# NetSys/demi

Measured on AMD Instinct MI355X. Metric: candidate schedules evaluated/sec on Raft-5 fuzz (RandomScheduler executions), higher is better.
Workload: dtype u8

## Files before the change

demi_amd/csrc/demi_device.hpp:

```cpp
#pragma once

#ifndef __HIPCC_RTC__
#include <hip/hip_runtime.h>
#include <stdint.h>
#endif

#include "../../include/demi_gpu.h"

namespace demi {

struct DevModel {
  uint32_t n_actors, n_msg_types, n_classes, code_len;
  uint32_t inv_kind, inv_fa, inv_va, inv_fb;
  uint32_t fp_match_mask, wide ;
  uint32_t n_timer_types;
  uint32_t timer_types;
  uint32_t meta[DEMI_MAX_MSG_TYPES];
  uint32_t handler_start[DEMI_MAX_CLASSES * DEMI_MAX_MSG_TYPES];
  uint32_t actor_class[DEMI_MAX_ACTORS];
  uint64_t init_state[DEMI_MAX_ACTORS];
  uint32_t divmagic[257];
  uint32_t arr_len;
  uint32_t optab[64];
  uint32_t code[DEMI_MAX_CODE];
// ... 125 lines not shown
__device__ __forceinline__ void pairs_clear(PairSet& p) { p.w = 0; }
__device__ __forceinline__ uint32_t pairs_get(const PairSet& p, uint32_t a, uint32_t b) { return (uint32_t)(p.w >> (a * 8 + b)) & 1u; }
__device__ __forceinline__ void pairs_put(PairSet& p, uint32_t a, uint32_t b, bool on) {
  if (on) p.w |= 1ULL << (a * 8 + b); else p.w &= ~(1ULL << (a * 8 + b));
}
#endif
struct Net {
  uint32_t inaccessible, killed;
  PairSet partitioned;
};
__device__ __forceinline__ bool crosses_partition(const Net& n, uint32_t snd, uint32_t rcv) {
  if (snd == rcv && !((n.killed >> snd) & 1)) return false;
#ifdef DEMI_BIG
  const uint32_t part = pairs_get(n.partitioned, snd, rcv) | pairs_get(n.partitioned, rcv, snd);
#else
  const uint32_t part = (uint32_t)((n.partitioned.w >> (snd * 8 + rcv)) | (n.partitioned.w >> (rcv * 8 + snd))) & 1u;
#endif
  return (part | (n.inaccessible >> rcv) | (n.inaccessible >> snd)) & 1u;
}

#ifdef DEMI_BIG
#ifndef DEMI_JIT_TYPE_OF_TIX
#define DEMI_JIT_TYPE_OF_TIX 0u
#endif
__device__ __forceinline__ uint32_t tq_pack(uint32_t rcv, uint32_t type, uint32_t tix) { (void)type; return (rcv << 2) | tix; }
__device__ __forceinline__ uint32_t tq_rcv(uint32_t b) { return b >> 2; }
__device__ __forceinline__ uint32_t tq_type(uint32_t b) { return ((uint32_t)(DEMI_JIT_TYPE_OF_TIX) >> (5u * (b & 3u))) & 31u; }
#else
__device__ __forceinline__ uint32_t tq_pack(uint32_t rcv, uint32_t type, uint32_t tix) { (void)tix; return (rcv << 5) | type; }
__device__ __forceinline__ uint32_t tq_rcv(uint32_t b) { return b >> 5; }
__device__ __forceinline__ uint32_t tq_type(uint32_t b) { return b & 31u; }
#endif

__device__ __forceinline__ void hash_step(uint64_t& h, uint64_t v) { h = (h ^ v) * 0x100000001B3ULL; }

__device__ __forceinline__ uint32_t fld(uint64_t s, uint32_t f) { return (uint32_t)(s >> (8 * f)) & 0xFF; }
__device__ __forceinline__ uint32_t state_field(const uint64_t* st, uint32_t a, uint32_t f) {
#ifdef DEMI_WIDE
  return (uint32_t)(st[(ST_WORDS * a + (f >> 2)) * 64] >> (16 * (f & 3))) & 0xFFFFu;
#else
  return (uint32_t)(st[(ST_WORDS * a) * 64] >> (8 * f)) & 0xFFu;
#endif
}
__device__ __forceinline__ uint32_t arr_load(const uint64_t* st, uint32_t a, uint32_t idx) {
  if (ARR_LEN == 0 || idx >= ARR_LEN) return 0;
  const unsigned char* w = reinterpret_cast<const unsigned char*>(st + (size_t)(ST_WORDS * a + FLD_WORDS + idx / (WIDE_TU ? 4u : 8u)) * 64);
  if (WIDE_TU) return reinterpret_cast<const uint16_t*>(w)[idx & 3u];
  return w[idx & 7u];
}
__device__ __forceinline__ void arr_store(uint64_t* st, uint32_t a, uint32_t idx, uint32_t v) {
  if (ARR_LEN == 0 || idx >= ARR_LEN) return;
  unsigned char* w = reinterpret_cast<unsigned char*>(st + (size_t)(ST_WORDS * a + FLD_WORDS + idx / (WIDE_TU ? 4u : 8u)) * 64);
  if (WIDE_TU) reinterpret_cast<uint16_t*>(w)[idx & 3u] = (uint16_t)v;
  else w[idx & 7u] = (unsigned char)v;
}


}
```

demi_amd/csrc/demi_gpu.hip:

```cpp
#include <hip/hip_runtime.h>

#include <cstdarg>
#include <cstdio>
#include <cstring>
#include <algorithm>
#include <memory>
#include <new>
#include <queue>
#include <string>
#include <type_traits>
#include <unordered_map>
#include <unordered_set>
#include <vector>
#include <chrono>

#include "../../include/demi_gpu.h"
#include "knobs.hpp"
#include "devbuf.hpp"
#include "k1_random_explore.hpp"
#include "k2_replay.hpp"
#include "k2_removal_round.hpp"
#include "k2_wildcard.hpp"
#include "k2_wildcard_cand.hpp"
#include "k2_wildcard_round.hpp"
// ... 548 lines not shown
  ctx->have_dpor = false;
  return DEMI_OK;
}

static bool is_big(const DevModel& h) { return h.n_actors > DEMI_MAX_ACTORS; }
static uint32_t jit_k1_hot();
static uint32_t jit_k1s_hot() {
  return demi_host::knob("DEMI_JIT_K1S_HOT") ? (uint32_t)demi_host::knob_int("DEMI_JIT_K1S_HOT", 0, 64, 0) : jit_k1_hot();
}
static uint32_t jit_k1_hot() {
  return (uint32_t)demi_host::knob_int("DEMI_JIT_K1_HOT", 0, 64, 0);
}

static uint32_t jit_k3_hot(const DevModel& h);
static std::string jit_source(const DevModel& h, int kernel) {
  std::string src =
      "typedef unsigned char uint8_t; typedef unsigned short uint16_t; typedef unsigned int uint32_t;\n"
      "typedef unsigned long uint64_t; typedef int int32_t; typedef long int64_t; typedef unsigned long size_t; typedef unsigned long uintptr_t;\n"
      "#include \"sim_core.hpp\"\n";
  char defs[512];
  snprintf(defs, sizeof defs, "#define DEMI_PEND_HOT %u\n#define DEMI_K1_HOT %u\n#define DEMI_JIT_A %uu\n#define DEMI_JIT_INV_KIND %uu\n#define DEMI_JIT_INV_FA %uu\n"
           "#define DEMI_JIT_INV_VA %uu\n#define DEMI_JIT_INV_FB %uu\n#define DEMI_JIT_FP_MASK 0x%xu\n"
           "#define DEMI_JIT_NTT %uu\n#define DEMI_JIT_TIMER_TYPES 0x%xu\n#define DEMI_JIT_TIX_PACKED 0x%llxull\n#define DEMI_JIT_NT %uu\n",
           (unsigned)(kernel == JK_K3 ? jit_k3_hot(h)  : h.wide ? DEMI_PEND_HOT / 2 : DEMI_PEND_HOT), (unsigned)((kJit[kernel].flags & JF_SPREAD) ? jit_k1s_hot() : jit_k1_hot()), h.n_actors, h.inv_kind, h.inv_fa, h.inv_va, h.inv_fb, h.fp_match_mask,
           h.n_timer_types, h.timer_types, (unsigned long long)h.tix_packed, h.n_msg_types);
  src = defs + src;
  if (h.inv_kind & DEMI_INV_PROGRAM) src = "#define DEMI_JIT_INV_PROG 1\n" + src;
  if (h.wide) src = "#define DEMI_WIDE 1\n" + src;
  if (is_big(h)) {
    uint32_t type_of_tix = 0;
    for (uint32_t t = 0; t < h.n_msg_types; t++) if ((h.timer_types >> t) & 1u) type_of_tix |= t << (5u * (h.meta[t] >> 8));
    src = "#define DEMI_BIG 1\n#define DEMI_JIT_TYPE_OF_TIX " + std::to_string(type_of_tix) + "u\n" + src;
  }
  if (h.npay > 2) src = "#define DEMI_JIT_NPAY " + std::to_string(h.npay) + "\n" + src;
  if (h.arr_len) src = "#define DEMI_JIT_ARR_LEN " + std::to_string(h.arr_len) + "u\n" + src;
  {
    bool crash = false, rnd = false;
    for (uint32_t pc = 0; pc < h.code_len; pc++) { crash |= (h.code[pc] & 0xFFu) == DEMI_OP_CRASH; rnd |= (h.code[pc] & 0x3Fu) == DEMI_OP_RND; }
    if (!crash) src = "#define DEMI_JIT_NO_CRASH 1\n" + src;
    if (!rnd) src = "#define DEMI_JIT_NO_RND 1\n" + src;
  }
  if (const char* d = demi_host::knob("DEMI_JIT_DEFINES")) {
    std::string extra, item;
    for (const char* c = d;; c++) {
      if (*c == ';' || *c == '\0') {
        if (!item.empty()) { const size_t eq = item.find('='); extra += "#define " + (eq == std::string::npos ? item : item.substr(0, eq) + " " + item.substr(eq + 1)) + "\n"; }
        item.clear();
        if (*c == '\0') break;
      } else item += *c;
    }
    src = extra + src;
  }
  if (const long x = demi_host::knob_int("DEMI_JIT_K1_WAVES_PER_EU", 1, 8, 0))
    src = "#define DEMI_K1_MIN_WAVES_PER_EU " + std::to_string(x) + "\n" + src;
  src += demi_jit::generate_vm(h, jk_is_k1(kernel) && !jk_k1_records(kernel) && !demi_host::knob("DEMI_JIT_NO_FX_SCHED"));
  src += "#define DEMI_VM_RUN vm_run_jit\n#include \"";
  src += kJit[kernel].include;
  src += "\"\n";
  if (kJit[kernel].args) src += std::string("template __global__ void ") + kJit[kernel].name + "(const " + kJit[kernel].args + ");\n";
  return src;
}

static int jit_compile(demi_ctx* ctx, const DevModel& h, int kernel, std::vector<char>& image, std::string& name) {
#ifdef DEMI_NO_JIT_SOURCES
  return fail(ctx, DEMI_ERR_DEVICE, "specialisation failed: this library was built without the embedded kernel sources "
                                    "(build it with __graft_entry__.build())");
// ... 3923 lines not shown
```

demi_amd/csrc/jit.hpp:

```cpp
#pragma once
#include "knobs.hpp"

#include <dlfcn.h>

#include <algorithm>
#include <cstdio>
#include <cstdlib>
#include <cstring>
#include <string>
#include <vector>

#include "sim_core.hpp"

namespace demi_jit {

struct FxSchedule {
  bool ok = false;
  std::vector<uint32_t> cls;
  std::vector<int32_t> slot;
};
enum : uint32_t { FXK_SEND = 0, FXK_CANCEL = 1, FXK_TSET = 2, FXK_CRASH = 3 };
inline uint32_t fx_class_of(uint32_t row) {
  const uint32_t op = row & 0x3Fu, type = (row >> 17) & 0x7Fu;
  if (op == DEMI_OP_SEND || op == DEMI_OP_BCAST) return FXK_SEND << 16;
// ... 135 lines not shown
    if (is_fx(pc)) {
      const uint32_t c = fx_class_of(h.code[pc]);
      int32_t j = next;
      while (j < (int32_t)S.cls.size() && S.cls[j] != c) j++;
      if (j >= (int32_t)S.cls.size()) { S.cls.push_back(c); j = (int32_t)S.cls.size() - 1; }
      S.slot[pc] = j;
      next = j + 1;
    }
    uint32_t o[2];
    const int k = succ(pc, o);
    for (int i = 0; i < k; i++) if (o[i] < n) lo[o[i]] = std::max(lo[o[i]], next);
  }
  {
    std::vector<int32_t> used(S.cls.size(), 0), remap(S.cls.size(), -1);
    for (uint32_t pc = 0; pc < n; pc++) if (S.slot[pc] >= 0) used[S.slot[pc]] = 1;
    std::vector<uint32_t> cls2;
    for (size_t j = 0; j < S.cls.size(); j++) if (used[j]) { remap[j] = (int32_t)cls2.size(); cls2.push_back(S.cls[j]); }
    for (uint32_t pc = 0; pc < n; pc++) if (S.slot[pc] >= 0) S.slot[pc] = remap[S.slot[pc]];
    S.cls.swap(cls2);
  }
  S.ok = S.cls.size() <= DEMI_FX_CAP;
  return S;
}

inline uint32_t k1_fxq_slots(const demi::DevModel& h, bool sched) {
  if (!sched) return DEMI_FX_CAP;
  const FxSchedule fxs = fx_schedule(h);
  if (!fxs.ok) return DEMI_FX_CAP;
  uint32_t nq = 0;
  for (uint32_t c : fxs.cls) nq += (c >> 16) == FXK_SEND;
  return nq ? nq : 1u;
}

inline std::string generate_vm(const demi::DevModel& h, bool sched = false) {
  using namespace demi;
  std::string s;
  char buf[512];
  auto emit = [&](const char* fmt, auto... a) { snprintf(buf, sizeof buf, fmt, a...); s += buf; };
  FxSchedule fxs;
  std::vector<uint32_t> fxq_of_slot;
  if (sched) fxs = fx_schedule(h);
  if (fxs.ok) {
    s += "#define DEMI_JIT_FX_SCHED 1\n#define DEMI_JIT_FX_APPLY";
    uint32_t nq = 0;
    for (size_t j = 0; j < fxs.cls.size(); j++) {
      const uint32_t c = fxs.cls[j], type = c & 0xFFu;
      const bool snd = (c >> 16) == FXK_SEND;
      emit(" DEMI_FX_SLOT(%zu, %uu, %uu, %uu, %uu, %uu)", j, c >> 16, (c >> 8) & 0xFFu, type, snd ? 0u : (h.meta[type & 31u] >> 8), snd ? nq : 0u);
      fxq_of_slot.push_back(snd ? nq : 0u);
      if (snd) nq++;
    }
    emit("\n#define DEMI_JIT_FXQ_SLOTS %uu\n", nq ? nq : 1u);
  }
  s += "namespace demi {\n";
  const bool long_msg = h.npay > 2;
  const char* fx_pack_fn = long_msg ? "fx_pack_area" : "fx_pack";
  if (fxs.ok)
    s += std::string("#define DEMI_FX_AT(SLOT, Q, OP, TYPE, TGT, ...) { mem.fxq[(Q) * 64] = ") + fx_pack_fn + "(OP, TYPE, TGT, __VA_ARGS__); nfx |= 1u << (SLOT); }\n"
         "#define DEMI_FX_MARK(SLOT) { nfx |= 1u << (SLOT); }\n";
  else
    s += std::string("#define DEMI_FX(OP, TYPE, TGT, ...) { if (nfx >= DEMI_FX_CAP) { flags |= DEMI_V_QUEUE_OVF; goto done; } "
         "mem.fxq[nfx * 64] = ") + fx_pack_fn + "(OP, TYPE, TGT, __VA_ARGS__); nfx++; }\n";
  const bool wide = h.wide != 0;
  const unsigned RM = wide ? 65535u : 255u, SM = wide ? 15u : 7u;
  emit("__device__ inline uint32_t vm_run_jit(const Tables& t, const LaneMem& mem, %s w, uint32_t& flags, uint64_t& app_rng) {\n",
       wide ? "word_t" : "uint32_t");
// ... 299 lines not shown
```

demi_amd/csrc/k1_random_explore.hpp:

```cpp
#pragma once

#include "sim_core.hpp"

#ifndef DEMI_VM_RUN
#define DEMI_VM_RUN vm_run
#endif

namespace demi {

struct K1Args {
  const DevModel* model;
  const uint64_t* trace;
  uint32_t n_ev;
  uint32_t exists;
  uint64_t seed_base;
  const uint64_t* seeds;
  uint64_t n;
  uint32_t max_messages, interval, looking_for_valid, looking_for;
  demi_verdict* out;
  unsigned long long* work_counter;
  uint32_t p_max;
  uint32_t* spill;
  demi_rec_event* rec_out;
  uint32_t* rec_count;
// ... 330 lines not shown
    __syncthreads();
  }
  auto td_ptr = [&](uint32_t e) -> unsigned char* { return tdir + ((e >> 2) << 8) + (e & 3u); };
#ifdef DEMI_JIT_NT
  constexpr bool TIX32 = DEMI_JIT_NT <= 16u;
#else
  constexpr bool TIX32 = false;
#endif
  auto tix_of = [&](uint32_t type) -> uint32_t {
    return TIX32 ? (((uint32_t)tix_packed >> (2 * type)) & 3u) : ((uint32_t)(tix_packed >> (2 * type)) & 3u);
  };
  auto timer_entry = [&](word_t pw, uint32_t& e) -> bool {
    const uint32_t ty = w_type(pw);
    e = w_dst(pw) * NTT + tix_of(ty);
    return w_src(pw) == DL && ((timer_types >> ty) & 1u);
  };
  const uint32_t E = t.E, exists = t.exists;
  const uint32_t max_messages = args.max_messages ? args.max_messages : 0x7FFFFFFFu;
  const uint32_t interval = args.interval;

  int ph = PH_IDLE;
  bool fresh = false;
  uint64_t sched = 0, rng = 0, hash = 0;
  uint64_t inst = 0, inst_end = 0;
  uint32_t exec_no = 0;
  uint64_t app_rng = 0;
  uint32_t n_pend = 0, count = 0, cnt_mod = 0, tidx = 0, inj_lo = 0, inj_hi = 0, batch_no = 0;
  uint32_t fl_off = 0, fl_cnt = 0;
  uint32_t n_norm = 0, n_pairs = 0;
  uint64_t pairmask = 0, te_rng = 0;
  Net net;
  net.inaccessible = 0; net.killed = 0; pairs_clear(net.partitioned);
  uint64_t reach = 0;
  uint64_t tq = 0, resend = 0;
  uint32_t n_tq = 0, n_resend = 0;
  tmask_t just = 0, rep = 0;
  auto reach_row = [&](uint32_t snd) -> uint32_t {
#ifdef DEMI_BIG
    return (s_batch[(size_t)(batch_no - 1u) * K1_BATCH_WORDS + 7u + (snd >> 1)] >> (16u * (snd & 1u))) & 0xFFFFu;
#else
    return (uint32_t)(reach >> (snd * 8)) & 0xFFu;
#endif
  };
  auto pair_has = [&](uint32_t pr) -> bool {
#ifdef DEMI_BIG
    bool h = false;
    for (uint32_t i = 0; i < n_pairs; i++) h |= pair_get(i) == pr;
    return h;
#else
    return (pairmask >> pr) & 1ull;
#endif
  };
  uint32_t viol = 0, flags = 0;
  uint32_t blocked = 0;
#ifdef DEMI_JIT_NO_CRASH
  constexpr bool CRASHES = false;
#else
  constexpr bool CRASHES = true;
#endif
  uint32_t hits = 0;
  word_t lastw = 0;
#ifdef DEMI_K1_NO_LASTW
#define LASTW() pend_load(mem, n_pend - 1)
#define LASTW_SET(W) do {} while (0)
#define LASTW_RELOAD() do {} while (0)
#else
#define LASTW() lastw
#define LASTW_SET(W) do { lastw = (W); } while (0)
#define LASTW_RELOAD() do { if (n_pend != 0) lastw = pend_load(mem, n_pend - 1); } while (0)
// ... 20 lines not shown
  } while (0)

#define PEND_APPEND(WORD, ID, TD_ENTRY)                               \
  do {                                                                \
    if (n_pend + n_norm >= PMAX) { flags |= DEMI_V_PENDING_OVF; }     \
    else {                                                            \
      pend_store(mem, n_pend, (WORD));                                \
      LASTW_SET(WORD);                                                \
      if (REC) aux_store(mem, n_pend, (ID));                          \
      if ((TD_ENTRY) >= 0) {                                          \
        unsigned char* const p_ = td_ptr((uint32_t)(TD_ENTRY));       \
        *p_ = (unsigned char)((*p_ == TD_NONE) ? n_pend : TD_MANY);   \
      }                                                               \
      n_pend++;                                                       \
    }                                                                 \
  } while (0)

#define NORM_APPEND(WORD, ID)                                         \
  do {                                                                \
    if (n_pend + n_norm >= PMAX) { flags |= DEMI_V_PENDING_OVF; }     \
    else {                                                            \
      const word_t w_ = (WORD);                                       \
      const uint32_t pr_ = w_src(w_) * MAX_ACT + w_dst(w_);           \
      norm_store(n_norm, w_);                                         \
      if (REC) norm_aux_store(n_norm, (ID));                          \
      if (!pair_has(pr_)) { pair_set(n_pairs, pr_); n_pairs++; if (!BIG_TU) pairmask |= 1ull << pr_; } \
      n_norm++;                                                       \
    }                                                                 \
  } while (0)

#define TIMER_BIT(RCV, TYPE) ((tmask_t)1 << ((RCV) * DEMI_MAX_TIMER_TYPES + tix_of(TYPE)))

  auto enqueue_timer = [&](uint32_t rcv, uint32_t type, tmask_t tbit) {
    const uint64_t b = (uint64_t)tq_pack(rcv, type, BIG_TU ? tix_of(type) : 0u);
    if (just & tbit) {
      if (n_resend >= DEMI_RESEND_CAP) { flags |= DEMI_V_QUEUE_OVF; return; }
      resend |= b << (8 * n_resend);
      n_resend++;
    } else {
      if (n_tq >= DEMI_TQ_CAP) { flags |= DEMI_V_QUEUE_OVF; return; }
      tq |= b << (8 * n_tq);
      n_tq++;
    }
  };

  auto pend_remove = [&](uint32_t idx, word_t rw, word_t lw) {
    const uint32_t last = n_pend - 1;
    pend_store(mem, idx, lw);
    if (REC) aux_store(mem, idx, aux_load(mem, last));
    uint32_t e;
    if (timer_entry(rw, e)) { unsigned char* const p = td_ptr(e); if (*p == idx) *p = (unsigned char)TD_NONE; }
    if (idx != last && timer_entry(lw, e)) { unsigned char* const p = td_ptr(e); if (*p == last) *p = (unsigned char)idx; }
    n_pend = last;
    LASTW_RELOAD();
  };
  auto tdir_rebuild = [&]() {
    for (uint32_t j = 0; j < k1_tdir_words(A, NTT); j++) *reinterpret_cast<uint32_t*>(tdir + (j << 8)) = 0xFFFFFFFFu;
    for (uint32_t q = 0; q < n_pend; q++) {
      uint32_t e;
      if (timer_entry(pend_load(mem, q), e)) { unsigned char* const p = td_ptr(e); *p = (unsigned char)((*p == TD_NONE) ? q : TD_MANY); }
    }
  };

#ifdef DEMI_JIT_A
  const uint32_t inv_kind = DEMI_JIT_INV_KIND, inv_fa = DEMI_JIT_INV_FA, inv_va = DEMI_JIT_INV_VA, inv_fb = DEMI_JIT_INV_FB,
                 fp_mask = DEMI_JIT_FP_MASK;
#else
  const uint32_t inv_kind = t.inv_kind, inv_fa = t.inv_fa, inv_va = t.inv_va, inv_fb = t.inv_fb, fp_mask = t.fp_mask;
#endif
  auto check_invariant = [&]() -> uint32_t {
    if (inv_kind & DEMI_INV_PEERS) {
      hits = 0;
      for (uint32_t a = 0; a < A; a++) if ((exists >> a) & 1u) hits |= invariant_hit_at(t, st, a, inv_kind, inv_fa, inv_va) << a;
    }
    const uint32_t fp = invariant_from_hits(t, st, hits & exists, A, inv_kind, inv_fb);
// ... 22 lines not shown
    bool service = true;
    if (DEMI_K1_SVC_PERIOD != 0) {
      const uint64_t waiting = __ballot(ph != PH_DISPATCH);
      service = (uint32_t)__popcll(waiting) >= (uint32_t)DEMI_K1_SVC_LANES || svc_age >= (uint32_t)DEMI_K1_SVC_PERIOD || waiting == ~0ull;
      svc_age = service ? 0u : svc_age + 1u;
    }
    if (service) {
      if (ph == PH_FINISH) {
        if (!(flags & (DEMI_OVF_ANY | DEMI_V_MAXMSG)) && !viol) viol = check_invariant();
        for (uint32_t i = 0; i < A * ST_WORDS; i++) hash_step(hash, st[i * 64]);
        uint4 v;
        if (flags & DEMI_OVF_ANY) {
          v.x = flags & DEMI_OVF_ANY; v.y = 0; v.z = 0; v.w = 0;
        } else {
          v.x = (flags & 0xFF) | (viol ? DEMI_V_VIOLATION : 0u) | ((tidx & 0xFF) << 8) | ((count < 0xFFFFu ? count : 0xFFFFu) << 16);
          v.y = viol; v.z = (uint32_t)hash; v.w = (uint32_t)(hash >> 32);
        }
        *reinterpret_cast<uint4*>(&args.out[sched]) = v;
        if (REC) args.rec_count[sched] = n_rec;
        if constexpr (MULTI) {
          const uint32_t cf = ((v.x & DEMI_V_VIOLATION) ? 1u : 0u) | ((v.x & DEMI_OVF_ANY) ? 2u : 0u);
          if (cf) atomicOr(&args.cand_flags[m_cand], cf);
        }
        if constexpr (TESTS) {
          const uint32_t cf = ((v.x & DEMI_V_VIOLATION) ? 1u : 0u) | ((v.x & DEMI_OVF_ANY) ? 2u : 0u);
          if (cf) atomicOr(&args.test_flags[m_cand], cf);
        }
        ph = PH_IDLE;
        if (CARRY && !(v.x & DEMI_V_VIOLATION) && sched + 1 < inst_end) {
          sched++; exec_no++;
          ph = PH_INJECT; fresh = true;
        }
        n_pend = 0; count = 0; cnt_mod = 0; tidx = 0; inj_lo = 0; inj_hi = 0; batch_no = 0;
        tq = 0; resend = 0; n_tq = 0; n_resend = 0; just = 0; rep = 0; viol = 0; flags = 0; hash = 0;
        n_norm = 0; n_pairs = 0; pairmask = 0;
      }
      PH_MARK(10);
      if constexpr (MULTI) {
        if (!exhausted) {
          exhausted = true;
          if (m_exec < args.epc && m_cand < args.n_cand) { ph = PH_INJECT; fresh = true; sched = (uint64_t)m_cand * args.epc + m_exec; }
        }
        if (__ballot(ph != PH_IDLE) == 0) break;
      } else if constexpr (TESTS) {
        if (!exhausted) {
          exhausted = true;
          if (m_exec < args.epc && m_cand < args.n_tests) { ph = PH_INJECT; fresh = true; sched = (uint64_t)m_cand * args.epc + m_exec; }
        }
        if (__ballot(ph != PH_IDLE) == 0) break;
      } else {
        uint32_t claim = K1_BATCH;
        bool may_claim = true;
        if constexpr (SPREAD) { claim = args.lanes_per_wave; may_claim = lane < args.lanes_per_wave; }
        const uint64_t idle = __ballot(ph == PH_IDLE && may_claim);
        if (idle != 0 && !exhausted) {
          const uint32_t want = (uint32_t)__popcll(idle);
          const uint64_t have = b_end - b_next;
          uint64_t got = 0;
          if (have < want) {
            if (lane == 0) got = atomicAdd(args.work_counter, (unsigned long long)claim);
            got = __shfl(got, 0);
          }
          if (ph == PH_IDLE && may_claim) {
            const uint32_t rank = (uint32_t)__popcll(idle & ((1ULL << lane) - 1));
            const uint64_t my = (rank < have) ? (b_next + rank) : (got + (rank - have));
            if (my < n_units) {
              ph = PH_INJECT; fresh = true;
// ... 104 lines not shown
        const uint32_t other = (uint32_t)__builtin_amdgcn_readlane((int)n_norm, src);
        for (uint32_t i = lane; i < cnt; i += 64) {
          const uint32_t slot = base + i;
          if (slot + other >= PMAX) break;
          const word_t sw = s_bsend[off + i];
          if (slot < K1_HOT) (mem.pend - lane + src)[slot * 64] = sw;
          else { *spill_at(mem.spill, __umul24(slot - K1_HOT, mem.spill_stride) + (mem.spill_lane - lane + (uint32_t)src)) = sw; spilled = true; }
        }
      }
#ifdef DEMI_K1_FLUSH_FENCE
      if (__ballot(spilled) != 0) __threadfence_block();
#else
      if (__ballot(spilled) != 0) __builtin_amdgcn_fence(__ATOMIC_RELEASE, "wavefront");
#endif
      if (step && fl_cnt != 0) {
        if (n_pend + n_norm + fl_cnt > PMAX) { flags |= DEMI_V_PENDING_OVF; n_pend = PMAX - n_norm; }
        else { n_pend += fl_cnt; LASTW_SET(s_bsend[fl_off + fl_cnt - 1]); }
        fl_cnt = 0;
      }
    }
    if (step) {
      if (REC) {
        for (uint32_t i = inj_lo; i < inj_hi; i++) {
          const word_t sw = s_sendw[i];
          if (sw != 0) {
            const uint32_t id = next_id; next_id++;
            PEND_APPEND(sw, id, -1);
            REC_PUSH(DEMI_REC_MSG_SEND, DL, w_dst(sw), w_type(sw), w_area(sw), 1, i, id);
          }
        }
        inj_lo = inj_hi;
      }
      for (uint32_t k = 0; k < n_tq; k++) {
        const uint32_t bt = (uint32_t)(tq >> (8 * k)) & 0xFF, rcv = tq_rcv(bt), type = tq_type(bt);
        const uint32_t id = next_id; if (REC) next_id++;
        const bool drop = (net.inaccessible >> rcv) & 1;
        if (!drop) PEND_APPEND(msg_word(type, DL, rcv, 0, 0), id, (int32_t)(rcv * NTT + tix_of(type)));
        REC_PUSH(DEMI_REC_MSG_SEND, DL, rcv, type, 0, 2 | (drop ? 4 : 0), 255, id);
      }
      tq = 0; n_tq = 0;
      if ((flags & DEMI_OVF_ANY) || n_pend + n_norm == 0) none = true;
    }
    PH_MARK(3);
    if (disp) {
      uint32_t wid = 0;
      auto fifo_dequeue = [&](uint32_t pi) {
        const uint32_t pr = pair_get(pi);
        uint32_t k = 0;
        word_t cur = norm_load(0);
        while (k + 1 < n_norm && w_src(cur) * MAX_ACT + w_dst(cur) != pr) { k++; cur = norm_load(k); }
        w = cur;
        if (REC) wid = norm_aux_load(k);
        bool more = false;
        for (uint32_t j = k; j + 1 < n_norm; j++) {
          const word_t nx = norm_load(j + 1);
          more |= (w_src(nx) * MAX_ACT + w_dst(nx) == pr);
          norm_store(j, nx);
          if (REC) norm_aux_store(j, norm_aux_load(j + 1));
        }
        n_norm--;
        if (!more) {
          for (uint32_t j = pi; j + 1 < n_pairs; j++) pair_set(j, pair_get(j + 1));
          n_pairs--;
          if (!BIG_TU) pairmask &= ~(1ull << pr);
        }
      };
      bool picked = false;
      if (CRASHES && !none && blocked != 0) {
        auto find_non_blocked = [&](uint64_t& g) -> bool {
          const uint32_t n0 = n_pend;
          uint32_t k = 0;
          bool found = false;
          while (n_pend > 0) {
// ... 51 lines not shown
      if (!none) {
        if (!picked) {
          bool from_te = true;
          uint32_t idx = 0;
          if (!FIFO) {
            idx = jr_next_int(rng, n_pend, t.magic);
          } else if (n_pairs == 0) {
            idx = jr_next_int(te_rng, n_pend, t.magic);
          } else {
            from_te = jr_next_int(rng, n_pend + n_norm, t.magic) < n_pend;
            if (from_te) idx = jr_next_int(te_rng, n_pend, t.magic);
          }
          if (from_te) {
            w = pend_load(mem, idx);
            if (REC) wid = aux_load(mem, idx);
            pend_remove(idx, w, LASTW());
          } else {
            fifo_dequeue(jr_next_int(rng, n_pairs, t.magic));
          }
        }
        count++;
        cnt_mod++; if (cnt_mod == interval) cnt_mod = 0;
        const uint32_t type = w_type(w), me = w_dst(w);
        REC_PUSH(DEMI_REC_MSG_EVENT, w_src(w), me, type, w_area(w), 0, 255, wid);
        hash_step(hash, w);
        const tmask_t tbit = TIMER_BIT(me, type);
        const bool is_rep = ((timer_types >> type) & 1u) && (rep & tbit);
        if (is_rep) {
          just |= tbit;
          enqueue_timer(me, type, tbit);
        } else {
          if (n_resend != 0) {
            if (n_tq + n_resend > DEMI_TQ_CAP) flags |= DEMI_V_QUEUE_OVF;
            else { tq |= resend << (8 * n_tq); n_tq += n_resend; }
          }
          resend = 0; n_resend = 0; just = 0;
        }
        deliver = !(flags & DEMI_OVF_ANY);
        if (!deliver) ph = PH_FINISH;
      } else {
        if ((flags & DEMI_OVF_ANY) || viol || tidx >= E) {
          ph = PH_FINISH;
        } else {
          REC_PUSH(DEMI_REC_QUIESCENCE, 0, 0, 0, 0, 0, 255, 0);
          ph = PH_INJECT;
        }
      }
    }

    PH_MARK(4);
    uint32_t rb_me = 0xFFu;
    uint32_t rb_owner = 0, rb_hit = 0;
    if (REBIN) {
      const uint32_t tid = threadIdx.x;
      uint32_t* const xo = rb_x + tid;
      uint32_t* const cnt = rb_cnt + rb_it * K1_RB_MAX_CLASSES;
      uint32_t k = 0;
      {
        const uint32_t me_ = w_dst(w);
        xo[k++ * RB_WG] = (flags & 0xFu) | (n_pend << 4) | (n_tq << 12) | (n_resend << 16) | (((uint32_t)(reach >> (me_ * 8)) & 0xFFu) << 20);
        xo[k++ * RB_WG] = (uint32_t)lastw; if (WIDE_TU) xo[k++ * RB_WG] = (uint32_t)((uint64_t)lastw >> 32);
        xo[k++ * RB_WG] = (uint32_t)tq; xo[k++ * RB_WG] = (uint32_t)(tq >> 32);
        xo[k++ * RB_WG] = (uint32_t)resend; xo[k++ * RB_WG] = (uint32_t)(resend >> 32);
        xo[k++ * RB_WG] = just; xo[k++ * RB_WG] = rep;
        if (RB_CRASHES) xo[k++ * RB_WG] = blocked;
        if (APP_RND) { xo[k++ * RB_WG] = (uint32_t)app_rng; xo[k++ * RB_WG] = (uint32_t)(app_rng >> 32); }
        if (deliver) {
          xo[k++ * RB_WG] = (uint32_t)w; if (WIDE_TU) xo[k++ * RB_WG] = (uint32_t)((uint64_t)w >> 32);
#ifdef DEMI_K1_RB_CLASS
          const uint32_t cls = (uint32_t)(DEMI_K1_RB_CLASS(w, (uint32_t)st[(ST_WORDS * me_) * 64])) & (K1_RB_MAX_CLASSES - 1u);
#else
          const uint32_t cls = w_type(w) & (K1_RB_MAX_CLASSES - 1u);
#endif
          const uint32_t pos = atomicAdd(&cnt[cls < RB_C ? cls : 0u], 1u);
          rb_list[(cls < RB_C ? cls : 0u) * RB_WG + pos] = (unsigned char)tid;
          rb_me = me_;
        }
      }
      if (lane == 0 && wave_live) rb_flag[rb_it] = 1u;
      __syncthreads();
      if (rb_flag[rb_it] == 0u) break;
      if (tid < K1_RB_MAX_CLASSES) rb_cnt[(rb_it ^ 1u) * K1_RB_MAX_CLASSES + tid] = 0u;
      if (tid == K1_RB_MAX_CLASSES) rb_flag[rb_it ^ 1u] = 0u;
      uint32_t acc = 0, base = 0, csel = 0;
      for (uint32_t c = 0; c < RB_C; c++) {
        const uint32_t n_c = cnt[c];
        if (tid >= acc) { csel = c; base = acc; }
        acc += n_c;
      }
      deliver = tid < acc;
      if (deliver) {
        const uint32_t o = rb_list[csel * RB_WG + (tid - base)];
        rb_owner = o;
        const uint32_t ow = o >> 6, ol = o & 63u;
        mem = lane_mem_carve(wave_base + (size_t)ow * lane_mem_wave_bytes(t.A, REC, K1_HOT, WIDE_TU, K1_FXQ_SLOTS), t.A, REC, ol, args.spill,
                             (size_t)blockIdx.x * blockDim.x + o, (size_t)gridDim.x * blockDim.x, K1_HOT);
        st = mem.st;
        tdir = tdir_base + (size_t)ow * k1_tdir_wave_bytes(t.A, t.n_timer_types) + (size_t)ol * 4;
        const uint32_t* const xi = rb_x + o;
        uint32_t j = 0;
        const uint32_t pk = xi[j++ * RB_WG];
        flags = pk & 0xFu; n_pend = (pk >> 4) & 0xFFu; n_tq = (pk >> 12) & 0xFu; n_resend = (pk >> 16) & 0xFu;
        { uint64_t lw = xi[j++ * RB_WG]; if (WIDE_TU) lw |= (uint64_t)xi[j++ * RB_WG] << 32; lastw = (word_t)lw; }
        tq = xi[j * RB_WG] | ((uint64_t)xi[(j + 1) * RB_WG] << 32); j += 2;
        resend = xi[j * RB_WG] | ((uint64_t)xi[(j + 1) * RB_WG] << 32); j += 2;
        just = xi[j++ * RB_WG]; rep = xi[j++ * RB_WG];
        if (RB_CRASHES) blocked = xi[j++ * RB_WG];
        if (APP_RND) { app_rng = xi[j * RB_WG] | ((uint64_t)xi[(j + 1) * RB_WG] << 32); j += 2; }
        { uint64_t mw = xi[j++ * RB_WG]; if (WIDE_TU) mw |= (uint64_t)xi[j++ * RB_WG] << 32; w = (word_t)mw; }
        reach = (uint64_t)((pk >> 20) & 0xFFu) << (w_dst(w) * 8);
      }
    }
    uint32_t nfx = 0;
    if (deliver) nfx = DEMI_VM_RUN(t, mem, w, flags, app_rng);
    if (deliver) {
      const uint32_t me_ = w_dst(w);
      if (!(inv_kind & DEMI_INV_PEERS)) {
        rb_hit = invariant_hit_at(t, st, me_, inv_kind, inv_fa, inv_va);
        if (!REBIN) hits = (hits & ~(1u << me_)) | (rb_hit << me_);
      }
    }
    PH_MARK(5);
#ifdef DEMI_K1_PHASES
    ph_iters++; ph_active += __popcll(__ballot(deliver));
#endif

    const uint32_t me = w_dst(w);
    auto send_targets = [&](uint32_t fx) -> uint32_t {
      const bool bc = ((fx & 31u) == DEMI_OP_BCAST);
      const uint32_t target = fx_target(fx);
      const uint32_t tm = bc ? ~(1u << me) : (1u << target);
      return tm & reach_row(me);
    };
    auto apply_send = [&](word_t fxw) {
      const uint32_t fx = (uint32_t)fxw;
      const uint32_t type = (fx >> 5) & 31u;
      if (REC) {
        const bool bc = ((fx & 31u) == DEMI_OP_BCAST);
        const uint32_t target = fx_target(fx);
        const uint32_t first = bc ? 0u : target, last = bc ? A : (target < A ? target + 1 : 0u);
        for (uint32_t r = first; r < last; r++) {
          if ((bc && r == me) || !((exists >> r) & 1)) continue;
          const uint32_t id = next_id; next_id++;
          const bool drop = crosses_partition(net, me, r);
          if (!drop) {
            if (FIFO) NORM_APPEND(fx_msg_word(fxw, type, me, r), id);
            else PEND_APPEND(fx_msg_word(fxw, type, me, r), id, -1);
          }
          REC_PUSH(DEMI_REC_MSG_SEND, me, r, type, fx_area(fxw), drop ? 4 : 0, 255, id);
        }
      } else {
        uint32_t tm = send_targets(fx);
        const word_t base = fx_msg_word(fxw, type, me, 0);
        while (tm) {
          const uint32_t r = (uint32_t)__builtin_ctz(tm);
          tm &= tm - 1;
          if (FIFO) NORM_APPEND(base | (r << 5), 0u);
          else PEND_APPEND(base | (r << 5), 0u, -1);
        }
      }
    };
    auto apply_cancel = [&](uint32_t type, tmask_t tbit, uint32_t tix) {
      rep &= ~tbit;
      const uint32_t want = tq_pack(me, type, tix);
      bool found = false;
      if (n_tq != 0) {
        const uint64_t x = tq ^ (0x0101010101010101ull * (uint64_t)want);
        uint64_t z = (x - 0x0101010101010101ull) & ~x & 0x8080808080808080ull;
        z &= (n_tq >= 8) ? ~0ull : ((1ull << (8 * n_tq)) - 1ull);
        if (z != 0) {
          const uint32_t q = (uint32_t)__builtin_ctzll(z) >> 3;
          const uint64_t lowm = (1ull << (8 * q)) - 1ull;
          tq = (tq & lowm) | ((tq >> 8) & ~lowm);
          n_tq--; found = true;
        }
      }
      if (!found) {
        unsigned char* const p = td_ptr(me * NTT + tix);
        const uint32_t d = *p;
        if (d != TD_NONE) {
          const word_t wantw = msg_word(type, DL, me, 0, 0);
          if (d != TD_MANY) {
            pend_remove(d, wantw, LASTW());
          } else {
            uint32_t first = 0xFFFFFFFFu, second = 0xFFFFFFFFu, copies = 0;
            for (uint32_t q = 0; q < n_pend; q++)
              if (pend_load(mem, q) == wantw) {
                if (copies == 0) first = q; else if (copies == 1) second = q;
                copies++;
              }
            if (copies != 0) {
              const uint32_t last = n_pend - 1;
              pend_remove(first, wantw, LASTW());
              if (copies == 2) *p = (unsigned char)(second == last ? first : second);
            }
            if (copies <= 1) *p = (unsigned char)TD_NONE;
          }
        }
      }
    };
    auto apply_timer_set = [&](bool repeating, uint32_t type, tmask_t bit) {
      if (!(rep & bit)) {
        if (repeating) rep |= bit;
        enqueue_timer(me, type, bit);
      }
    };
    if (deliver) {
#ifdef DEMI_JIT_FX_SCHED
#define DEMI_FX_SLOT(J, KIND, OP, TYPE, TIDX, Q)                                                                      \
      if (((nfx >> (J)) & 1u) && !(flags & DEMI_OVF_ANY)) {                                                           \
        if ((KIND) == 0u) apply_send(mem.fxq[(Q) * 64]);                      \
        else if ((KIND) == 1u) apply_cancel((TYPE), (tmask_t)1 << (me * DEMI_MAX_TIMER_TYPES + (TIDX)), (TIDX));               \
        else if ((KIND) == 2u) apply_timer_set((OP) == DEMI_OP_TREP, (TYPE), (tmask_t)1 << (me * DEMI_MAX_TIMER_TYPES + (TIDX))); \
        else if (CRASHES) blocked |= 1u << me;                                                                        \
      }                                                                                                               \
      PH_MARK((KIND) == 0u ? 6 : (KIND) == 1u ? 7 : 8);
      DEMI_JIT_FX_APPLY
#undef DEMI_FX_SLOT
#else
      for (uint32_t k = 0; k < nfx && !(flags & DEMI_OVF_ANY); k++) {
        const word_t fxw = mem.fxq[k * 64];
        const uint32_t fx = (uint32_t)fxw;
        const uint32_t op = fx & 31u, type = (fx >> 5) & 31u;
        PH_MARK(9);
        if (op <= DEMI_OP_BCAST) { apply_send(fxw); PH_MARK(6); }
        else if (op == DEMI_OP_CRASH) { if (CRASHES) blocked |= 1u << me; }
        else if (op == DEMI_OP_TCANCEL) { apply_cancel(type, TIMER_BIT(me, type), tix_of(type)); PH_MARK(7); }
        else { apply_timer_set(op == DEMI_OP_TREP, type, TIMER_BIT(me, type)); PH_MARK(8); }
      }
#endif
      if (!REBIN && (flags & DEMI_OVF_ANY)) ph = PH_FINISH;
    }
    if (REBIN) {
      if (deliver) {
        uint32_t* const xb = rb_x + rb_owner;
        uint32_t k = 0;
        xb[k++ * RB_WG] = (flags & 0xFu) | (n_pend << 4) | (n_tq << 12) | (n_resend << 16) | (rb_hit << 28);
        xb[k++ * RB_WG] = (uint32_t)lastw; if (WIDE_TU) xb[k++ * RB_WG] = (uint32_t)((uint64_t)lastw >> 32);
        xb[k++ * RB_WG] = (uint32_t)tq; xb[k++ * RB_WG] = (uint32_t)(tq >> 32);
        xb[k++ * RB_WG] = (uint32_t)resend; xb[k++ * RB_WG] = (uint32_t)(resend >> 32);
        xb[k++ * RB_WG] = just; xb[k++ * RB_WG] = rep;
        if (RB_CRASHES) xb[k++ * RB_WG] = blocked;
        if (APP_RND) { xb[k++ * RB_WG] = (uint32_t)app_rng; xb[k++ * RB_WG] = (uint32_t)(app_rng >> 32); }
      }
      __syncthreads();
      {
        const uint32_t* const xi = rb_x + threadIdx.x;
        uint32_t j = 0;
        const uint32_t pk = xi[j++ * RB_WG];
        flags = pk & 0xFu; n_pend = (pk >> 4) & 0xFFu; n_tq = (pk >> 12) & 0xFu; n_resend = (pk >> 16) & 0xFu;
        { uint64_t lw = xi[j++ * RB_WG]; if (WIDE_TU) lw |= (uint64_t)xi[j++ * RB_WG] << 32; lastw = (word_t)lw; }
        tq = xi[j * RB_WG] | ((uint64_t)xi[(j + 1) * RB_WG] << 32); j += 2;
        resend = xi[j * RB_WG] | ((uint64_t)xi[(j + 1) * RB_WG] << 32); j += 2;
        just = xi[j++ * RB_WG]; rep = xi[j++ * RB_WG];
        if (RB_CRASHES) blocked = xi[j++ * RB_WG];
        if (APP_RND) { app_rng = xi[j * RB_WG] | ((uint64_t)xi[(j + 1) * RB_WG] << 32); j += 2; }
        if (rb_me != 0xFFu) {
          hits = (hits & ~(1u << rb_me)) | (((pk >> 28) & 1u) << rb_me);
          if (flags & DEMI_OVF_ANY) ph = PH_FINISH;
        }
      }
      mem = own_mem; st = own_mem.st; tdir = own_tdir;
      if (batch_no != 0) {
        const uint32_t* bt = s_batch + (size_t)(batch_no - 1) * K1_BATCH_WORDS;
        reach = (uint64_t)bt[7] | ((uint64_t)bt[8] << 32);
      }
      rb_it ^= 1u;
    }

    PH_MARK(9);
  }
#ifdef DEMI_K1_PHASES
  PH_MARK(11);
  if (lane == 0 && args.phase_out) {
    unsigned long long* o = args.phase_out + ((size_t)blockIdx.x * K1_WAVES + wave) * 16;
    for (int i = 0; i < 12; i++) o[i] = ph_t[i];
    o[14] = ph_iters; o[15] = ph_active;
  }
#endif
#undef PH_MARK
#undef REC_PUSH
#undef PEND_APPEND
#undef NORM_APPEND
#undef LASTW
#undef LASTW_SET
#undef LASTW_RELOAD
// ... 5 lines not shown
```

Before: 326.5 million.

## Pack timer queue into 4-bit entries and track queued timers with a bitmask

Introduces a TimerQ abstraction. When the JIT detects few actors times timer types (at most 16), the queue is stored in a 32-bit word with 4-bit entries instead of a 64-bit word of bytes, and each entry's type is decoded from a JIT constant. It also keeps an 'inq' bitmask of which timers sit in the queue, so timer cancel can skip the SWAR search when the timer is absent. This lowers register pressure and ALU work per event, at the cost of more code paths and per-model JIT defines.

```diff
diff --git a/demi_amd/csrc/demi_device.hpp b/demi_amd/csrc/demi_device.hpp
--- a/demi_amd/csrc/demi_device.hpp
+++ b/demi_amd/csrc/demi_device.hpp
@@ -181,6 +181,46 @@
 __device__ __forceinline__ uint32_t tq_type(uint32_t b) { return b & 31u; }
 #endif
 
+#if defined(DEMI_JIT_TQ4_TYPES) && !defined(DEMI_BIG) && !defined(DEMI_K1_TQ_BYTES)
+constexpr bool TQ_NARROW = true;
+struct TimerQ {
+  typedef uint32_t bits_t;
+  static constexpr uint32_t W = 4;
+  static constexpr bits_t ONES = 0x11111111u;
+  bits_t bits;
+  static __device__ __forceinline__ uint32_t pack(uint32_t rcv, uint32_t type, uint32_t tix) { (void)type; return rcv * (DEMI_JIT_NTT) + tix; }
+  static __device__ __forceinline__ uint32_t rcv_of(uint32_t e) { return e / (DEMI_JIT_NTT); }
+  static __device__ __forceinline__ uint32_t type_of(uint32_t e) { return ((uint32_t)(DEMI_JIT_TQ4_TYPES) >> (5u * (e % (DEMI_JIT_NTT)))) & 31u; }
+  static __device__ __forceinline__ bits_t splat(uint32_t e) { bits_t r = e | (e << 4); r |= r << 8; return r | (r << 16); }
+#else
+constexpr bool TQ_NARROW = false;
+struct TimerQ {
+  typedef uint64_t bits_t;
+  static constexpr uint32_t W = 8;
+  static constexpr bits_t ONES = 0x0101010101010101ull;
+  bits_t bits;
+  static __device__ __forceinline__ uint32_t pack(uint32_t rcv, uint32_t type, uint32_t tix) { return tq_pack(rcv, type, tix); }
+  static __device__ __forceinline__ uint32_t rcv_of(uint32_t e) { return tq_rcv(e); }
+  static __device__ __forceinline__ uint32_t type_of(uint32_t e) { return tq_type(e); }
+  static __device__ __forceinline__ bits_t splat(uint32_t e) { return ONES * (bits_t)e; }
+#endif
+  static constexpr uint32_t CAP = 8 * sizeof(bits_t) / W;
+  __device__ __forceinline__ void clear() { bits = 0; }
+  __device__ __forceinline__ void push(uint32_t n, uint32_t e) { bits |= (bits_t)e << (W * n); }
+  __device__ __forceinline__ void append(uint32_t n, const TimerQ& o) { bits |= o.bits << (W * n); }
+  __device__ __forceinline__ uint32_t at(uint32_t k) const { return (uint32_t)(bits >> (W * k)) & ((1u << W) - 1u); }
+  __device__ __forceinline__ bool remove_first(uint32_t n, uint32_t e) {
+    const bits_t x = bits ^ splat(e);
+    bits_t z = (x - ONES) & ~x & (ONES << (W - 1));
+    z &= (n >= CAP) ? ~(bits_t)0 : (((bits_t)1 << (W * n)) - (bits_t)1);
+    if (z == 0) return false;
+    const uint32_t q = (uint32_t)(sizeof(bits_t) == 8 ? __builtin_ctzll(z) : __builtin_ctz((uint32_t)z)) / W;
+    const bits_t lowm = ((bits_t)1 << (W * q)) - (bits_t)1;
+    bits = (bits & lowm) | ((bits >> W) & ~lowm);
+    return true;
+  }
+};
+
 __device__ __forceinline__ void hash_step(uint64_t& h, uint64_t v) { h = (h ^ v) * 0x100000001B3ULL; }
 
 __device__ __forceinline__ uint32_t fld(uint64_t s, uint32_t f) { return (uint32_t)(s >> (8 * f)) & 0xFF; }
diff --git a/demi_amd/csrc/demi_gpu.hip b/demi_amd/csrc/demi_gpu.hip
--- a/demi_amd/csrc/demi_gpu.hip
+++ b/demi_amd/csrc/demi_gpu.hip
@@ -604,6 +604,7 @@
     for (uint32_t t = 0; t < h.n_msg_types; t++) if ((h.timer_types >> t) & 1u) type_of_tix |= t << (5u * (h.meta[t] >> 8));
     src = "#define DEMI_BIG 1\n#define DEMI_JIT_TYPE_OF_TIX " + std::to_string(type_of_tix) + "u\n" + src;
   }
+  src = demi_jit::tq_defines(h) + src;
   if (h.npay > 2) src = "#define DEMI_JIT_NPAY " + std::to_string(h.npay) + "\n" + src;
   if (h.arr_len) src = "#define DEMI_JIT_ARR_LEN " + std::to_string(h.arr_len) + "u\n" + src;
   {
diff --git a/demi_amd/csrc/jit.hpp b/demi_amd/csrc/jit.hpp
--- a/demi_amd/csrc/jit.hpp
+++ b/demi_amd/csrc/jit.hpp
@@ -191,6 +191,16 @@
   return nq ? nq : 1u;
 }
 
+inline std::string tq_defines(const demi::DevModel& h) {
+  if (h.n_actors > DEMI_MAX_ACTORS || h.n_timer_types == 0 || h.n_actors * h.n_timer_types > 16) return "";
+  uint32_t type_of_tix = 0;
+  for (uint32_t t = 0; t < h.n_msg_types; t++)
+    if ((h.timer_types >> t) & 1u) type_of_tix |= t << (5u * ((h.meta[t] >> 8) & 3u));
+  char buf[64];
+  snprintf(buf, sizeof buf, "#define DEMI_JIT_TQ4_TYPES 0x%xu\n", type_of_tix);
+  return buf;
+}
+
 inline std::string generate_vm(const demi::DevModel& h, bool sched = false) {
   using namespace demi;
   std::string s;
diff --git a/demi_amd/csrc/k1_random_explore.hpp b/demi_amd/csrc/k1_random_explore.hpp
--- a/demi_amd/csrc/k1_random_explore.hpp
+++ b/demi_amd/csrc/k1_random_explore.hpp
@@ -386,9 +386,15 @@
   Net net;
   net.inaccessible = 0; net.killed = 0; pairs_clear(net.partitioned);
   uint64_t reach = 0;
-  uint64_t tq = 0, resend = 0;
+  TimerQ tq = {0}, resend = {0};
   uint32_t n_tq = 0, n_resend = 0;
   tmask_t just = 0, rep = 0;
+  tmask_t inq = 0;
+#ifdef DEMI_K1_NO_INQ
+  constexpr bool INQ = false;
+#else
+  constexpr bool INQ = !REBIN;
+#endif
   auto reach_row = [&](uint32_t snd) -> uint32_t {
 #ifdef DEMI_BIG
     return (s_batch[(size_t)(batch_no - 1u) * K1_BATCH_WORDS + 7u + (snd >> 1)] >> (16u * (snd & 1u))) & 0xFFFFu;
@@ -475,15 +481,16 @@
 #define TIMER_BIT(RCV, TYPE) ((tmask_t)1 << ((RCV) * DEMI_MAX_TIMER_TYPES + tix_of(TYPE)))
 
   auto enqueue_timer = [&](uint32_t rcv, uint32_t type, tmask_t tbit) {
-    const uint64_t b = (uint64_t)tq_pack(rcv, type, BIG_TU ? tix_of(type) : 0u);
+    const uint32_t b = TimerQ::pack(rcv, type, (BIG_TU || TQ_NARROW) ? tix_of(type) : 0u);
     if (just & tbit) {
       if (n_resend >= DEMI_RESEND_CAP) { flags |= DEMI_V_QUEUE_OVF; return; }
-      resend |= b << (8 * n_resend);
+      resend.push(n_resend, b);
       n_resend++;
     } else {
       if (n_tq >= DEMI_TQ_CAP) { flags |= DEMI_V_QUEUE_OVF; return; }
-      tq |= b << (8 * n_tq);
+      tq.push(n_tq, b);
       n_tq++;
+      if (INQ) inq |= tbit;
     }
   };
 
@@ -572,7 +579,7 @@
           ph = PH_INJECT; fresh = true;
         }
         n_pend = 0; count = 0; cnt_mod = 0; tidx = 0; inj_lo = 0; inj_hi = 0; batch_no = 0;
-        tq = 0; resend = 0; n_tq = 0; n_resend = 0; just = 0; rep = 0; viol = 0; flags = 0; hash = 0;
+        tq.clear(); resend.clear(); n_tq = 0; n_resend = 0; just = 0; rep = 0; inq = 0; viol = 0; flags = 0; hash = 0;
         n_norm = 0; n_pairs = 0; pairmask = 0;
       }
       PH_MARK(10);
@@ -743,13 +750,13 @@
         inj_lo = inj_hi;
       }
       for (uint32_t k = 0; k < n_tq; k++) {
-        const uint32_t bt = (uint32_t)(tq >> (8 * k)) & 0xFF, rcv = tq_rcv(bt), type = tq_type(bt);
+        const uint32_t bt = tq.at(k), rcv = TimerQ::rcv_of(bt), type = TimerQ::type_of(bt);
         const uint32_t id = next_id; if (REC) next_id++;
         const bool drop = (net.inaccessible >> rcv) & 1;
-        if (!drop) PEND_APPEND(msg_word(type, DL, rcv, 0, 0), id, (int32_t)(rcv * NTT + tix_of(type)));
+        if (!drop) PEND_APPEND(msg_word(type, DL, rcv, 0, 0), id, (int32_t)(TQ_NARROW ? bt : rcv * NTT + tix_of(type)));
         REC_PUSH(DEMI_REC_MSG_SEND, DL, rcv, type, 0, 2 | (drop ? 4 : 0), 255, id);
       }
-      tq = 0; n_tq = 0;
+      tq.clear(); n_tq = 0; inq = 0;
       if ((flags & DEMI_OVF_ANY) || n_pend + n_norm == 0) none = true;
     }
     PH_MARK(3);
@@ -867,9 +874,9 @@
         } else {
           if (n_resend != 0) {
             if (n_tq + n_resend > DEMI_TQ_CAP) flags |= DEMI_V_QUEUE_OVF;
-            else { tq |= resend << (8 * n_tq); n_tq += n_resend; }
-          }
-          resend = 0; n_resend = 0; just = 0;
+            else { tq.append(n_tq, resend); n_tq += n_resend; if (INQ) inq |= just; }
+          }
+          resend.clear(); n_resend = 0; just = 0;
         }
         deliver = !(flags & DEMI_OVF_ANY);
         if (!deliver) ph = PH_FINISH;
@@ -895,8 +902,8 @@
         const uint32_t me_ = w_dst(w);
         xo[k++ * RB_WG] = (flags & 0xFu) | (n_pend << 4) | (n_tq << 12) | (n_resend << 16) | (((uint32_t)(reach >> (me_ * 8)) & 0xFFu) << 20);
         xo[k++ * RB_WG] = (uint32_t)lastw; if (WIDE_TU) xo[k++ * RB_WG] = (uint32_t)((uint64_t)lastw >> 32);
-        xo[k++ * RB_WG] = (uint32_t)tq; xo[k++ * RB_WG] = (uint32_t)(tq >> 32);
-        xo[k++ * RB_WG] = (uint32_t)resend; xo[k++ * RB_WG] = (uint32_t)(resend >> 32);
+        xo[k++ * RB_WG] = (uint32_t)tq.bits; xo[k++ * RB_WG] = (uint32_t)((uint64_t)tq.bits >> 32);
+        xo[k++ * RB_WG] = (uint32_t)resend.bits; xo[k++ * RB_WG] = (uint32_t)((uint64_t)resend.bits >> 32);
         xo[k++ * RB_WG] = just; xo[k++ * RB_WG] = rep;
         if (RB_CRASHES) xo[k++ * RB_WG] = blocked;
         if (APP_RND) { xo[k++ * RB_WG] = (uint32_t)app_rng; xo[k++ * RB_WG] = (uint32_t)(app_rng >> 32); }
@@ -937,8 +944,8 @@
         const uint32_t pk = xi[j++ * RB_WG];
         flags = pk & 0xFu; n_pend = (pk >> 4) & 0xFFu; n_tq = (pk >> 12) & 0xFu; n_resend = (pk >> 16) & 0xFu;
         { uint64_t lw = xi[j++ * RB_WG]; if (WIDE_TU) lw |= (uint64_t)xi[j++ * RB_WG] << 32; lastw = (word_t)lw; }
-        tq = xi[j * RB_WG] | ((uint64_t)xi[(j + 1) * RB_WG] << 32); j += 2;
-        resend = xi[j * RB_WG] | ((uint64_t)xi[(j + 1) * RB_WG] << 32); j += 2;
+        tq.bits = (TimerQ::bits_t)(xi[j * RB_WG] | ((uint64_t)xi[(j + 1) * RB_WG] << 32)); j += 2;
+        resend.bits = (TimerQ::bits_t)(xi[j * RB_WG] | ((uint64_t)xi[(j + 1) * RB_WG] << 32)); j += 2;
         just = xi[j++ * RB_WG]; rep = xi[j++ * RB_WG];
         if (RB_CRASHES) blocked = xi[j++ * RB_WG];
         if (APP_RND) { app_rng = xi[j * RB_WG] | ((uint64_t)xi[(j + 1) * RB_WG] << 32); j += 2; }
@@ -997,18 +1004,9 @@
     };
     auto apply_cancel = [&](uint32_t type, tmask_t tbit, uint32_t tix) {
       rep &= ~tbit;
-      const uint32_t want = tq_pack(me, type, tix);
       bool found = false;
-      if (n_tq != 0) {
-        const uint64_t x = tq ^ (0x0101010101010101ull * (uint64_t)want);
-        uint64_t z = (x - 0x0101010101010101ull) & ~x & 0x8080808080808080ull;
-        z &= (n_tq >= 8) ? ~0ull : ((1ull << (8 * n_tq)) - 1ull);
-        if (z != 0) {
-          const uint32_t q = (uint32_t)__builtin_ctzll(z) >> 3;
-          const uint64_t lowm = (1ull << (8 * q)) - 1ull;
-          tq = (tq & lowm) | ((tq >> 8) & ~lowm);
-          n_tq--; found = true;
-        }
+      if (INQ ? (inq & tbit) != 0 : n_tq != 0) {
+        if (tq.remove_first(n_tq, TimerQ::pack(me, type, tix))) { n_tq--; found = true; }
       }
       if (!found) {
         unsigned char* const p = td_ptr(me * NTT + tix);
@@ -1072,8 +1070,8 @@
         uint32_t k = 0;
         xb[k++ * RB_WG] = (flags & 0xFu) | (n_pend << 4) | (n_tq << 12) | (n_resend << 16) | (rb_hit << 28);
         xb[k++ * RB_WG] = (uint32_t)lastw; if (WIDE_TU) xb[k++ * RB_WG] = (uint32_t)((uint64_t)lastw >> 32);
-        xb[k++ * RB_WG] = (uint32_t)tq; xb[k++ * RB_WG] = (uint32_t)(tq >> 32);
-        xb[k++ * RB_WG] = (uint32_t)resend; xb[k++ * RB_WG] = (uint32_t)(resend >> 32);
+        xb[k++ * RB_WG] = (uint32_t)tq.bits; xb[k++ * RB_WG] = (uint32_t)((uint64_t)tq.bits >> 32);
+        xb[k++ * RB_WG] = (uint32_t)resend.bits; xb[k++ * RB_WG] = (uint32_t)((uint64_t)resend.bits >> 32);
         xb[k++ * RB_WG] = just; xb[k++ * RB_WG] = rep;
         if (RB_CRASHES) xb[k++ * RB_WG] = blocked;
         if (APP_RND) { xb[k++ * RB_WG] = (uint32_t)app_rng; xb[k++ * RB_WG] = (uint32_t)(app_rng >> 32); }
@@ -1085,8 +1083,8 @@
         const uint32_t pk = xi[j++ * RB_WG];
         flags = pk & 0xFu; n_pend = (pk >> 4) & 0xFFu; n_tq = (pk >> 12) & 0xFu; n_resend = (pk >> 16) & 0xFu;
         { uint64_t lw = xi[j++ * RB_WG]; if (WIDE_TU) lw |= (uint64_t)xi[j++ * RB_WG] << 32; lastw = (word_t)lw; }
-        tq = xi[j * RB_WG] | ((uint64_t)xi[(j + 1) * RB_WG] << 32); j += 2;
-        resend = xi[j * RB_WG] | ((uint64_t)xi[(j + 1) * RB_WG] << 32); j += 2;
+        tq.bits = (TimerQ::bits_t)(xi[j * RB_WG] | ((uint64_t)xi[(j + 1) * RB_WG] << 32)); j += 2;
+        resend.bits = (TimerQ::bits_t)(xi[j * RB_WG] | ((uint64_t)xi[(j + 1) * RB_WG] << 32)); j += 2;
         just = xi[j++ * RB_WG]; rep = xi[j++ * RB_WG];
         if (RB_CRASHES) blocked = xi[j++ * RB_WG];
         if (APP_RND) { app_rng = xi[j * RB_WG] | ((uint64_t)xi[(j + 1) * RB_WG] << 32); j += 2; }
```

Result: faster. 334.2 million, median of 6 (+2.3%).
